# pecos/tps

Hardware: AMD Instinct MI355X
Metric: DG RHS evals/sec (MDOF/s) for 3D p=3 reacting cyl at 1/2/4/8 MI355X (higher is better)
Workload: dtype f64

## Files before the change

tps_amd/csrc/kernels.hpp:

```cpp
#ifndef TPSRHS_KERNELS_HPP_
#define TPSRHS_KERNELS_HPP_

#include <hip/hip_runtime.h>

#include <type_traits>

#include "basis.hpp"
#include "physics_dryair.hpp"

namespace tpsrhs {

#ifndef TPSRHS_MINW_GRAD
#define TPSRHS_MINW_GRAD 1
#endif
#ifndef TPSRHS_MINW_FLUX
#define TPSRHS_MINW_FLUX 3
#endif
#ifndef TPSRHS_NT_STORES
#define TPSRHS_NT_STORES 0
#endif
#ifndef TPSRHS_NO_MFMA
#define TPSRHS_NO_MFMA 0
#endif
#ifndef TPSRHS_FLUX_LATE
#define TPSRHS_FLUX_LATE 0
#endif
#ifndef TPSRHS_ABLATE
#define TPSRHS_ABLATE 0
#endif
constexpr int cmax(int a, int b) { return a > b ? a : b; }

#ifndef TPSRHS_STAMP
#define TPSRHS_STAMP 0
#endif
#if TPSRHS_STAMP
constexpr int NSTAMP = 16, STAMP_BLOCKS = 1 << 16;
static __device__ unsigned int g_stamp[STAMP_BLOCKS][NSTAMP];
struct Stamper {
  unsigned long long t0;
  unsigned int acc[NSTAMP];
  __device__ inline unsigned long long now() {
    unsigned long long t;
    __builtin_amdgcn_sched_barrier(0);
    asm volatile("s_memtime %0\n\ts_waitcnt lgkmcnt(0)" : "=s"(t)::"memory");
    __builtin_amdgcn_sched_barrier(0);
    return t;
  }
  __device__ inline void start() {
    for (int i = 0; i < NSTAMP; i++) acc[i] = 0;
    t0 = now();
  }
  __device__ inline void mark(int phase) {
    const unsigned long long t = now();
    acc[phase] += static_cast<unsigned int>(t - t0);
    t0 = t;
  }
  __device__ inline void flush() {
    if (threadIdx.x == 0 && blockIdx.x < STAMP_BLOCKS)
      for (int i = 0; i < NSTAMP; i++) g_stamp[blockIdx.x][i] = acc[i];
  }
};
#endif
#ifndef TPSRHS_DUMPF
#define TPSRHS_DUMPF 0
#endif
#if TPSRHS_DUMPF
constexpr int DUMPF_MAX = 1 << 22;
static __device__ double g_dumpf[DUMPF_MAX];
#endif
#if TPSRHS_STAMP == 1
#define STAMP_DECL Stamper stamper
#define STAMP_ARG , stamper
#define STAMP_PARAM , Stamper &stamper
#define STAMP_START() stamper.start()
#define STAMP(phase) stamper.mark(phase)
#define STAMP_FLUSH() stamper.flush()
#else
#define STAMP_DECL
#define STAMP_ARG
#define STAMP_PARAM
#define STAMP_START()
#define STAMP(phase)
#define STAMP_FLUSH()
#endif
#if TPSRHS_STAMP == 2
#define FSTAMP_DECL \
  Stamper stamper;  \
  stamper.start()
#define FSTAMP(phase) stamper.mark(phase)
#define FSTAMP_FLUSH() stamper.flush()
#else
#define FSTAMP_DECL
#define FSTAMP(phase)
#define FSTAMP_FLUSH()
#endif

static __constant__ Tables1D c_tab[2][2][TPSRHS_MAXORDER + 1];

__device__ inline const Tables1D &fresh_table(const Tables1D &ct) {
  typedef const Tables1D __attribute__((address_space(4))) *CP;
  const unsigned long long a = reinterpret_cast<unsigned long long>(&ct);
  unsigned lo = __builtin_amdgcn_readfirstlane(static_cast<unsigned>(a));
  unsigned hi = __builtin_amdgcn_readfirstlane(static_cast<unsigned>(a >> 32));
  asm volatile("" : "+s"(lo), "+s"(hi));
  return *(const Tables1D *)reinterpret_cast<CP>((static_cast<unsigned long long>(hi) << 32) | lo);
}

__device__ inline double ldsr(const double *p) { return *p; }

__device__ inline const double *field_ptr(const double *base, int k, int64_t stride) { return base + k * stride; }
__device__ inline double *field_ptr(double *base, int k, int64_t stride) { return base + k * stride; }

template <int BLOCK>
__device__ inline void block_sync() {
  if (BLOCK == 64) {
    __builtin_amdgcn_fence(__ATOMIC_RELEASE, "wavefront");
    __builtin_amdgcn_wave_barrier();
    __builtin_amdgcn_fence(__ATOMIC_ACQUIRE, "wavefront");
  } else {
    __syncthreads();
  }
}

template <int DIM_, int P_, int NC_ = 0>
struct Cfg {
  static constexpr int DIM = DIM_, P = P_, N1 = P_ + 1, NC = NC_;
  static constexpr int NPE = (DIM_ == 3) ? N1 * N1 * N1 : N1 * N1;
  static constexpr int NF = (DIM_ == 3) ? N1 * N1 : N1;
  static constexpr int Q1 = ((DIM_ - 1) + 2 * P_) / 2 + 1 + NC_;
  static constexpr int QV = P_ + 1 + NC_;
  static constexpr int NQV = (DIM_ == 3) ? QV * QV * QV : QV * QV;
  static constexpr int NQ = (DIM_ == 3) ? Q1 * Q1 : Q1;
  static constexpr int NW = (DIM_ == 3) ? Q1 * N1 : 1;
  static constexpr int NFACES = 2 * DIM_;
  static constexpr int NV = 1 << DIM_;
  static constexpr int BLOCK = (NC_ && DIM_ == 3 && P_ >= 2) ? 128 : ((NPE <= 64) ? 64 : ((NPE <= 128) ? 128 : 256));
  static constexpr int EPB = (DIM_ == 3 && NC_) ? (P_ == 3 ? 1 : 2)
                             : (DIM_ == 3 && P_ == 1) ? 3
                             : (DIM_ == 2 && NC_ && P_ == 1) ? 10
                                                             : BLOCK / NPE;
  static constexpr int NODES = EPB * NPE;
  static constexpr int PF = 2 * EPB;
  static constexpr int TN = PF * NF;
  static constexpr int TW = PF * NW;
  static constexpr int TQ = PF * NQ;
  static constexpr int LN = EPB * NF;
  static constexpr int Q_ROUNDS = (TQ + BLOCK - 1) / BLOCK;
  static_assert(DIM_ == 2 || Q_ROUNDS == 1, "3-D: one round of face quadrature points per direction pair");
  static_assert(!(DIM_ == 2 && NC_) || Q_ROUNDS == 1, "2-D Gauss-Lobatto pair: one round per direction pair");
  static constexpr int TQ2 = 2 * TQ;
  static constexpr int Q2_ROUNDS = (TQ2 + BLOCK - 1) / BLOCK;
};

template <class C>
struct Tab {
  double x[C::N1], w[C::N1], iw[C::N1], D[C::N1 * C::N1], b0[C::N1], b1[C::N1];
  double xq[C::Q1], wq[C::Q1], B[C::Q1 * C::N1];
  double xv[C::QV], wv[C::QV];
};

struct ForcingDev {
  int has_pg, nheat, nsponge, pad;
  double pg[3];
  struct Heat {
    double value, radius, len;
    double p1[3], axis[3];
  } heat[TPSRHS_MAXHEATSOURCES];
  struct Sponge {
    int type, pad;
    double normal[3], p0[3], pinit[3];
    double r1, r2, mult;
    double target[TPSRHS_MAXEQUATIONS];
    int mixed_out, n_plane;
    const int *plane_nodes;
    double *msum;
  } sponge[TPSRHS_MAXSPONGEZONES];
  const double *joule;
  int nps, pad2;
  struct Scalar {
    double x0[3], radius, value;
  } ps[TPSRHS_MAXPASSIVESCALARS];
// ... 1177 lines not shown
      for (int eq = 1; eq < NEQ; eq++) out[(eq - 1) * C::NQ] = fn[eq];
    }
    STAMP(8);
  }
}
template <class C, class PH, int D, int CD>
__device__ inline void lean_grad_chunk(const double *sJ, double *Tb, double *Wb, const Tab<C> &tab, const Tables1D &ct0,
                                       const double *n, double *gv, double *gn, int tid) {
  constexpr int NEQ = PH::NEQ, DIM = C::DIM, NVEL = PH::NVEL;
  const Tables1D &ct = fresh_table(ct0);
  trace_lines<C, D, NEQ>(sJ, Tb, ct, tid);
  block_sync<C::BLOCK>();
  interp1_lines<C, NEQ>(Tb, Wb, ct, tid);
  block_sync<C::BLOCK>();
  if (tid < C::TQ) {
    const int pf = tid / C::NQ, q = tid - pf * C::NQ;
    double bq[C::N1];
#pragma unroll
    for (int a = 0; a < C::N1; a++) bq[a] = tab.B[(q / C::Q1) * C::N1 + a];
#pragma unroll
    for (int k = 0; k < NEQ; k++) {
      const double val = interp2_point<C>(Tb + k * C::TN, Wb + k * C::TW, bq, pf, q);
      if (k >= 1 && k <= NVEL)
        gv[(k - 1) + CD * DIM] = val;
      else
        gn[k] += n[CD] * val;
    }
  }
  block_sync<C::BLOCK>();
}
template <class C, class PH, int D>
__device__ inline void lean_grad_dir(const MeshDev &m, const double *gradUp_q, bool node_on, unsigned node, double *gnext, double *sJ,
                                     double *Tb, double *Wb, const Tab<C> &tab, const Tables1D &ct, const double *n, double *gv,
                                     double *gn, int tid) {
  constexpr int NEQ = PH::NEQ;
  auto stage = [&](auto ctag) {
    constexpr int CD = decltype(ctag)::value;
    if (node_on) {
#pragma unroll
      for (int eq = 0; eq < NEQ; eq++) sJ[eq * C::NODES + tid] = gnext[eq];
      if (CD + 1 < C::DIM) {
        unsigned nq = node;
        int64_t stride = m.ndofs;
        asm volatile("" : "+v"(nq), "+s"(stride));
#pragma unroll
        for (int eq = 0; eq < NEQ; eq++) gnext[eq] = field_ptr(gradUp_q, (CD + 1) * NEQ + eq, stride)[nq];
      }
    }
    block_sync<C::BLOCK>();
    lean_grad_chunk<C, PH, D, CD>(sJ, Tb, Wb, tab, ct, n, gv, gn, tid);
  };
  stage(std::integral_constant<int, 0>());
  stage(std::integral_constant<int, 1>());
  stage(std::integral_constant<int, 2>());
}
template <class C, class PH>
__device__ inline void visc_phase_lean3d(const MeshDev &m, const int2 *sFI, typename PH::PRef prm0, int e0, const double *sU,
                                         const double *gradUp_q, bool node_on, unsigned node, double *sJ, double *Tb, double *Wb,
                                         const double *sV, const Tab<C> &tab, const Tables1D &ct, double *__restrict__ TB,
                                         int tid0 STAMP_PARAM) {
  constexpr int NEQ = PH::NEQ, DIM = C::DIM;
  static_assert(DIM == 3 && C::Q_ROUNDS == 1 && PH::NVEL == 3 && C::BLOCK == 64, "3-D, one wave, one round of face points per pair");
#pragma clang loop unroll(disable)
  for (int d = 0; d < DIM; d++) {
    typename PH::PRef prm = PH::relaunder(prm0);
    int tid = tid0;
    asm volatile("" : "+v"(tid));
    const int pf = tid / C::NQ, q = tid - pf * C::NQ;
    const int le = pf >> 1, s = pf & 1;
    const bool on = tid < C::TQ && (e0 + le) < m.ne;
    int nb = 0;
    double n[DIM] = {1.0, 0.0, 0.0};
    if (on) {
      double wq, Xq[DIM];
      nb = sFI[le * C::NFACES + 2 * d + s].x;
      face_geometry_rt<C>(d, &sV[le * C::NV * DIM], tab, s, q, n, wq, Xq);
    }
    const int np_lane = on ? PH::visc_passes(prm, nb) : 0;
    const int npass = (__ballot(np_lane == 2) != 0) ? 2 : ((__ballot(np_lane >= 1) != 0) ? 1 : 0);
    double *out = TB + static_cast<int64_t>((e0 + le) * C::NFACES + 2 * d + s) * ((NEQ - 1) * C::NQ) + q;
    if (on && np_lane == 0) {
#pragma unroll
      for (int eq = 1; eq < NEQ; eq++) out[(eq - 1) * C::NQ] = 0.0;
    }
#pragma clang loop unroll(disable)
    for (int pass = 0; pass < npass; pass++) {
      double u[NEQ];
#pragma unroll
      for (int k = 0; k < NEQ; k++) u[k] = 1.0;
      if (d == 0)
        visc_state_dir<C, PH, 0>(sU, Tb, Wb, tab, ct, u, tid);
      else if (d == 1)
        visc_state_dir<C, PH, 1>(sU, Tb, Wb, tab, ct, u, tid);
      else
        visc_state_dir<C, PH, 2>(sU, Tb, Wb, tab, ct, u, tid);
      STAMP(5);
      PH::clamp_species(u);
      double gnext[NEQ];
#pragma unroll
      for (int eq = 0; eq < NEQ; eq++) gnext[eq] = 0.0;
      if (node_on) {
        unsigned nq = node;
        int64_t stride = m.ndofs;
        asm volatile("" : "+v"(nq), "+s"(stride));
#pragma unroll
        for (int eq = 0; eq < NEQ; eq++) gnext[eq] = field_ptr(gradUp_q, eq, stride)[nq];
      }
      typename PH::ViscLean cf;
      if (pass < np_lane) {
        typename PH::PRef pq = PH::relaunder(prm);
        double Us[NEQ];
        typename PH::WallFlux w;
        PH::visc_pass_state(pq, nb, pass, u, n, Us, w);
        PH::visc_point_lean(pq, Us, w, cf);
      }
      STAMP(6);
      double gv[DIM * DIM], gn[NEQ];
#pragma unroll
      for (int k = 0; k < DIM * DIM; k++) gv[k] = 0.0;
#pragma unroll
      for (int eq = 0; eq < NEQ; eq++) gn[eq] = 0.0;
      if (d == 0)
        lean_grad_dir<C, PH, 0>(m, gradUp_q, node_on, node, gnext, sJ, Tb, Wb, tab, ct, n, gv, gn, tid);
      else if (d == 1)
        lean_grad_dir<C, PH, 1>(m, gradUp_q, node_on, node, gnext, sJ, Tb, Wb, tab, ct, n, gv, gn, tid);
      else
        lean_grad_dir<C, PH, 2>(m, gradUp_q, node_on, node, gnext, sJ, Tb, Wb, tab, ct, n, gv, gn, tid);
      STAMP(7);
      if (pass < np_lane) {
        double f[NEQ];
        PH::visc_normal_flux_lean(cf, gv, gn, n, f);
        if (nb >= 0) {
#pragma unroll
          for (int eq = 1; eq < NEQ; eq++) {
            if (TPSRHS_NT_STORES)
              __builtin_nontemporal_store(f[eq], &out[(eq - 1) * C::NQ]);
            else
              out[(eq - 1) * C::NQ] = f[eq];
          }
        } else if (pass == 0) {
#pragma unroll
          for (int eq = 1; eq < NEQ; eq++) out[(eq - 1) * C::NQ] = -0.5 * f[eq];
        } else {
#pragma unroll
          for (int eq = 1; eq < NEQ; eq++) out[(eq - 1) * C::NQ] -= 0.5 * f[eq];
        }
      }
      STAMP(8);
    }
    if (on && npass == 0) {
    }
  }
}
template <class C, class PH>
__device__ inline void visc_phase_2d(const MeshDev &m, const int2 *sFI, typename PH::PRef prm, int e0,
                                     const double *sU, const double *g, bool node_on, double *sJ, double *Tb,
                                     const double *sV, const Tab<C> &tab, const Tables1D &ct, double *__restrict__ TB,
                                     int tid, const double *sDist = nullptr) {
  static_assert(C::DIM == 2, "2-D only");
  constexpr int NEQ = PH::NEQ;
  typedef GradLds<C, PH> L;
  constexpr int G0 = PH::VISC_USES_GRAD_RHO ? 0 : 1, NG = NEQ - G0;
  double v[C::Q2_ROUNDS][L::NVF];
  auto chunk = [&](auto nfld_tag, const double *src, int v0) {
    constexpr int NF_ = decltype(nfld_tag)::value;
    trace_lines<C, 0, NF_>(src, Tb, ct, tid);
    trace_lines<C, 1, NF_>(src, Tb + L::CH * C::TN, ct, tid);
    block_sync<C::BLOCK>();
#pragma unroll
    for (int rd = 0; rd < C::Q2_ROUNDS; rd++) {
      int item = tid + rd * C::BLOCK;
      if (item < C::TQ2) {
        const int d = item / C::TQ;
        item -= d * C::TQ;
        const int pf = item / C::NQ, q = item - pf * C::NQ;
        const double *T = Tb + d * (L::CH * C::TN);
        double bq[C::N1];
#pragma unroll
        for (int a = 0; a < C::N1; a++) bq[a] = tab.B[q * C::N1 + a];
#pragma unroll
        for (int k = 0; k < NF_; k++) v[rd][v0 + k] = interp2_point<C>(T + k * C::TN, nullptr, bq, pf, q);
      }
    }
    block_sync<C::BLOCK>();
  };
  chunk(std::integral_constant<int, NEQ>(), sU, 0);
  FaceDist<C::Q2_ROUNDS> dq;
  dq.on = sDist != nullptr;
  if (sDist) {
    trace_lines<C, 0, 1>(sDist, Tb, ct, tid);
    trace_lines<C, 1, 1>(sDist, Tb + L::CH * C::TN, ct, tid);
    block_sync<C::BLOCK>();
#pragma unroll
    for (int rd = 0; rd < C::Q2_ROUNDS; rd++) {
      int item = tid + rd * C::BLOCK;
      dq.d[rd] = 0.0;
      if (item < C::TQ2) {
        const int d = item / C::TQ;
        item -= d * C::TQ;
        const int pf = item / C::NQ, q = item - pf * C::NQ;
        double bq[C::N1];
#pragma unroll
        for (int a = 0; a < C::N1; a++) bq[a] = tab.B[q * C::N1 + a];
        dq.d[rd] = interp2_point<C>(Tb + d * (L::CH * C::TN), nullptr, bq, pf, q);
      }
    }
    block_sync<C::BLOCK>();
  }
#pragma unroll
  for (int c = 1; c <= 2; c++) {
    const double *src;
    if constexpr (L::G_IN_LDS) {
      src = sJ + ((c - 1) * NEQ + G0) * C::NODES;
    } else {
      if (node_on) {
#pragma unroll
        for (int eq = G0; eq < NEQ; eq++) sJ[eq * C::NODES + tid] = g[eq + (c - 1) * NEQ];
      }
      block_sync<C::BLOCK>();
      src = sJ + G0 * C::NODES;
    }
    if (G0) {
#pragma unroll
      for (int rd = 0; rd < C::Q2_ROUNDS; rd++) v[rd][c * NEQ] = 0.0;
    }
    chunk(std::integral_constant<int, NG>(), src, c * NEQ + G0);
  }
  visc_points<C, PH, true>(m, sFI, prm, e0, 0, v, sV, tab, TB, tid, dq);
}
template <class C, class PH, int D>
__device__ inline void visc_traces_dir(const MeshDev &m, const int2 *sFI, typename PH::PRef prm, int e0,
                                       const double *sU, const double *g, bool node_on, double *sJ, double *Tb, double *Wb,
                                       const double *sV, const Tab<C> &tab, const Tables1D &ct, double *__restrict__ TB,
                                       int tid) {
  double v[C::Q_ROUNDS][GradLds<C, PH>::NVF];
  visc_interp_dir<C, PH, D>(sU, g, node_on, sJ, Tb, Wb, tab, ct, v, tid);
  visc_points<C, PH>(m, sFI, prm, e0, D, v, sV, tab, TB, tid);
}

template <class C, class PH>
__global__ __launch_bounds__(C::BLOCK, (C::NC && PH::HEAVY) ? 1 : PH::minw_grad(C::DIM, C::P, C::NC)) void k_gradient(MeshDev m, typename PH::KArg prm_k,
                                                       const double *__restrict__ U, const double *__restrict__ TA,
                                                       double *__restrict__ Upout, double *__restrict__ gradUp,
                                                       double *__restrict__ TB) {
  typename PH::PRef prm = PH::pref(prm_k);
  constexpr int NEQ = PH::NEQ, DIM = C::DIM;
  typedef GradLds<C, PH> L;
  const Tables1D &ct = c_tab[C::NC][DIM - 2][C::P];
  __shared__ Tab<C> tab;
  __shared__ double sV[C::EPB * C::NV * DIM];
  __shared__ double pool[L::TOTAL];
  double *sU = pool + L::O_U;
  double *sUp = pool + L::O_UP;
  double *sJ = pool + L::O_J;
  double *sW = pool + L::O_W;

  const int tid = threadIdx.x;
  const int lin = xcd_block(static_cast<int>(blockIdx.x), static_cast<int>(gridDim.x), m.reverse);
  const int bid = m.blocks ? m.blocks[lin] : lin;
  const int e0 = (TPSRHS_ABLATE & 512) ? (bid % 8) * C::EPB : bid * C::EPB;
  __shared__ int2 sFI[C::EPB * C::NFACES];
  STAMP_DECL;
  STAMP_START();
  const bool node_on = tid < C::NODES && (e0 + tid / C::NPE) < m.ne;
  const int le_n = tid / C::NPE, nd = tid - le_n * C::NPE;
  int idx[3] = {nd % C::N1, (nd / C::N1) % C::N1, nd / (C::N1 * C::N1)};
  double u[NEQ];
  if (node_on) {
    const unsigned n = static_cast<unsigned>(e0 + le_n) * C::NPE + nd;
#pragma unroll
    for (int eq = 0; eq < NEQ; eq++) u[eq] = field_ptr(U, eq, m.ndofs)[n];
  }
  load_face_info<C>(sFI, m, e0);
  load_tables<C>(tab, ct);
  load_vertices<C>(sV, m, e0);
  block_sync<C::BLOCK>();
  STAMP(0);
  NbTraces<C, NEQ> ta0, ta1, ta2;
  constexpr bool LATE = TPSRHS_GRAD_LATE && ((DIM == 3 && (!C::NC || TPSRHS_GRAD_LATE_NC) && !PH::HEAVY) || TPSRHS_GRAD_LATE_ALL);
  issue_neighbour_traces<C, 0, NEQ>(sFI, TA, 2 * NEQ * C::NF, NEQ, ta0, tid);
  if (!LATE) {
    issue_neighbour_traces<C, 1, NEQ>(sFI, TA, 2 * NEQ * C::NF, NEQ, ta1, tid);
    if (DIM == 3) issue_neighbour_traces<C, (DIM == 3 ? 2 : 0), NEQ>(sFI, TA, 2 * NEQ * C::NF, NEQ, ta2, tid);
  }
  if (node_on) {
    const unsigned n = static_cast<unsigned>(e0 + le_n) * C::NPE + nd;
    double up[NEQ];
    PH::prim(prm, u, up);
#pragma unroll
    for (int eq = 0; eq < NEQ; eq++) {
      sU[eq * C::NODES + tid] = u[eq];
      sUp[eq * C::NODES + tid] = up[eq];
      if (TPSRHS_NT_STORES)
        __builtin_nontemporal_store(up[eq], &field_ptr(Upout, eq, m.ndofs)[n]);
      else
        field_ptr(Upout, eq, m.ndofs)[n] = up[eq];
    }
  }
  block_sync<C::BLOCK>();
  STAMP(1);

  double g[NEQ * DIM];
#pragma unroll
  for (int k = 0; k < NEQ * DIM; k++) g[k] = 0.0;
  double inv_mass = 0.0;
  if constexpr (C::NC) {
    nc_volume_gradient<C, NEQ>(sUp, pool + L::O_V, sV, tab, ct, node_on, le_n, nd, tid, g);
  } else if (node_on) {
    double xi[DIM], J[DIM * DIM], A[DIM * DIM];
    double iwn = 1.0;
#pragma unroll
    for (int d = 0; d < DIM; d++) {
      xi[d] = tab.x[idx[d]];
      iwn *= tab.iw[idx[d]];
    }
    jacobian<DIM>(&sV[le_n * C::NV * DIM], xi, J);
    const double det = adjugate<DIM>(J, A);
    const double idet = fast_rcp(det);
    inv_mass = iwn * idet;
    double Dr[DIM][C::N1];
#pragma unroll
    for (int mm = 0; mm < DIM; mm++)
#pragma unroll
      for (int a = 0; a < C::N1; a++) Dr[mm][a] = tab.D[idx[mm] * C::N1 + a];
#pragma unroll
    for (int eq = 0; eq < NEQ; eq++) {
      double dr[DIM];
#pragma unroll
      for (int mm = 0; mm < DIM; mm++) {
        const int m2 = ((TPSRHS_ABLATE & 128) && DIM == 3) ? 2 : mm;
        const int sd = stride_of<C>(m2);
        const double *F = &sUp[eq * C::NODES + le_n * C::NPE + nd - idx[m2] * sd];
        double acc = 0.0;
#pragma unroll
        for (int a = 0; a < C::N1; a++) acc += Dr[mm][a] * ldsr(&F[a * sd]);
        dr[mm] = acc;
      }
#pragma unroll
      for (int d = 0; d < DIM; d++) {
        double s = 0.0;
#pragma unroll
        for (int mm = 0; mm < DIM; mm++) s += A[mm + d * DIM] * dr[mm];
        g[eq + d * NEQ] = s * idet;
      }
    }
  }

  STAMP(2);
  if (!(TPSRHS_ABLATE & 8)) {
    auto jump = [&](auto dtag) {
      constexpr int D = decltype(dtag)::value;
      if constexpr (C::NC) {
        nc_grad_jump<C, PH, D>(sFI, prm, sJ, pool + L::O_V, sV, tab, ct, node_on, le_n, idx, tid, g);
      } else {
        if (node_on) grad_jump_nodal<C, PH>(D, sFI, prm, sJ, sJ + NEQ * C::TN, sV, tab, le_n, idx, inv_mass, g);
        block_sync<C::BLOCK>();
      }
    };
    if (LATE) issue_neighbour_traces<C, 1, NEQ>(sFI, TA, 2 * NEQ * C::NF, NEQ, ta1, tid);
    trace_lines<C, 0, NEQ>(sUp, sJ, ct, tid);
    block_sync<C::BLOCK>();
    store_neighbour_traces<C, NEQ>(ta0, sJ, sJ + NEQ * C::TN, tid);
    block_sync<C::BLOCK>();
    jump(std::integral_constant<int, 0>());
    if (LATE && DIM == 3) issue_neighbour_traces<C, (DIM == 3 ? 2 : 0), NEQ>(sFI, TA, 2 * NEQ * C::NF, NEQ, ta2, tid);
    trace_lines<C, 1, NEQ>(sUp, sJ, ct, tid);
    block_sync<C::BLOCK>();
    store_neighbour_traces<C, NEQ>(ta1, sJ, sJ + NEQ * C::TN, tid);
    block_sync<C::BLOCK>();
    jump(std::integral_constant<int, 1>());
    if (DIM == 3) {
      trace_lines<C, (DIM == 3 ? 2 : 0), NEQ>(sUp, sJ, ct, tid);
      block_sync<C::BLOCK>();
      store_neighbour_traces<C, NEQ>(ta2, sJ, sJ + NEQ * C::TN, tid);
      block_sync<C::BLOCK>();
      jump(std::integral_constant<int, (DIM == 3 ? 2 : 0)>());
    }
  }
  if constexpr (C::NC) {
    if constexpr (C::NPE == 64 && C::BLOCK == 128 && !TPSRHS_NO_MFMA) {
      static_assert(L::V >= 64 * 17, "LDS buffer of the MFMA inverse mass");
      nc_apply_minv_mfma<C, NEQ * DIM>(m.minv, pool + L::O_V, node_on, e0, nd, tid, g);
    }
    else
      nc_apply_minv<C, NEQ * DIM>(m.minv, pool + L::O_V, node_on, e0 + le_n, le_n, nd, tid, g);
  }

  STAMP(3);
  if (node_on) {
    const unsigned n = static_cast<unsigned>(e0 + le_n) * C::NPE + nd;
#pragma unroll
    for (int k = 0; k < NEQ * DIM; k++) field_ptr(gradUp, k, m.ndofs)[n] = g[k];
    if constexpr (L::G_IN_LDS) {
#pragma unroll
      for (int k = 0; k < NEQ * DIM; k++) sJ[k * C::NODES + tid] = g[k];
    }
  }
  if (L::G_IN_LDS) block_sync<C::BLOCK>();
  STAMP(4);
  if constexpr (L::LEAN3D) {
    if (!(TPSRHS_ABLATE & 16)) {
      asm volatile("s_waitcnt vmcnt(0)" ::: "memory");
      const double *gq = gradUp;
      const unsigned node = static_cast<unsigned>(e0 + le_n) * C::NPE + nd;
      visc_phase_lean3d<C, PH>(m, sFI, prm, e0, sU, gq, node_on, node, sJ, sUp, sW, sV, tab, ct, TB, tid STAMP_ARG);
    }
    STAMP_FLUSH();
    return;
  }

  if (!(TPSRHS_ABLATE & 16)) {
    if constexpr (DIM == 2) {
      if constexpr (PH::HEAVY) {
        __shared__ double sDist[C::NODES];
        const bool ml_on = m.ml.distance != nullptr;
        if (ml_on) {
          if (tid < C::NODES)
            sDist[tid] = node_on ? m.ml.distance[static_cast<int64_t>(e0 + le_n) * C::NPE + nd] : 0.0;
          block_sync<C::BLOCK>();
        }
        visc_phase_2d<C, PH>(m, sFI, prm, e0, sU, g, node_on, sJ, sUp, sV, tab, ct, TB, tid, ml_on ? sDist : nullptr);
      } else {
        visc_phase_2d<C, PH>(m, sFI, prm, e0, sU, g, node_on, sJ, sUp, sV, tab, ct, TB, tid);
      }
    } else if constexpr (PH::TWO_STEP && C::Q_ROUNDS == 1 && !(TPSRHS_ABLATE & 256)) {
      visc_phase_heavy3d<C, PH>(m, sFI, prm, e0, sU, sJ, sUp, sW, sV, tab, ct, TB, tid STAMP_ARG);
    } else if constexpr (PH::HEAVY) {
#pragma clang loop unroll(disable)
      for (int d = 0; d < DIM; d++) {
        double v[C::Q_ROUNDS][L::NVF];
        if (d == 0)
          visc_interp_dir<C, PH, 0>(sU, g, node_on, sJ, sUp, sW, tab, ct, v, tid);
        else if (d == 1)
          visc_interp_dir<C, PH, 1>(sU, g, node_on, sJ, sUp, sW, tab, ct, v, tid);
        else
          visc_interp_dir<C, PH, (DIM == 3 ? 2 : 0)>(sU, g, node_on, sJ, sUp, sW, tab, ct, v, tid);
        visc_points<C, PH>(m, sFI, prm, e0, d, v, sV, tab, TB, tid);
      }
    } else {
      visc_traces_dir<C, PH, 0>(m, sFI, prm, e0, sU, g, node_on, sJ, sUp, sW, sV, tab, ct, TB, tid);
      visc_traces_dir<C, PH, 1>(m, sFI, prm, e0, sU, g, node_on, sJ, sUp, sW, sV, tab, ct, TB, tid);
      if (DIM == 3)
        visc_traces_dir<C, PH, (DIM == 3 ? 2 : 0)>(m, sFI, prm, e0, sU, g, node_on, sJ, sUp, sW, sV, tab, ct, TB, tid);
    }
  }
  STAMP_FLUSH();
}

template <class C, class PH>
__device__ inline void apply_forcing(const ForcingDev &f, typename PH::PRef prm, int64_t node, const double *X,
                                     const double *u, const typename PH::State &st, const double *gr, double *src) {
  constexpr int NEQ = PH::NEQ, DIM = C::DIM, NVEL = PH::NVEL;
  if (f.has_pg) {
    double gpv = 0.0;
#pragma unroll
    for (int d = 0; d < DIM; d++) {
      src[1 + d] -= f.pg[d];
      gpv -= st.vel[d] * f.pg[d];
      gpv -= st.p * gr[(1 + d) + d * NEQ];
    }
    src[1 + NVEL] += gpv;
  }
  if (f.nps > 0) {
    double up[NEQ];
    PH::prim(prm, u, up);
    for (int i = 0; i < f.nps; i++) {
      const ForcingDev::Scalar &ps = f.ps[i];
      double dist = 0.0;
#pragma unroll
      for (int d = 0; d < DIM; d++) dist += (X[d] - ps.x0[d]) * (X[d] - ps.x0[d]);
      if (sqrt(dist) < ps.radius) {
        double vel = 0.0;
#pragma unroll
        for (int d = 0; d < DIM; d++) vel += up[1 + d] * up[1 + d];
        vel = sqrt(vel);
        src[NEQ - 1] -= vel * (up[NEQ - 1] - up[0] * ps.value) / ps.radius;
      }
    }
  }
  for (int z = 0; z < f.nsponge; z++) {
    const ForcingDev::Sponge &sz = f.sponge[z];
    double dist_init = 0.0, dist_f = 0.0;
#pragma unroll
    for (int d = 0; d < DIM; d++) {
      dist_init -= sz.normal[d] * (X[d] - sz.pinit[d]);
      dist_f += sz.normal[d] * (X[d] - sz.p0[d]);
    }
    double sigma = 0.0;
    double tgt[NEQ];
#pragma unroll
    for (int eq = 0; eq < NEQ; eq++) tgt[eq] = sz.target[eq];
    if (sz.type == TPSRHS_SPONGE_PLANAR) {
      if (dist_init > 0.0 && dist_f > 0.0) {
        const double len = dist_f + dist_init;
        sigma = dist_init / len / len;
      }
    } else if constexpr (DIM == 3) {
      double t[3], R = 0.0;
#pragma unroll
      for (int d = 0; d < 3; d++) {
        t[d] = X[d] - sz.pinit[d] + dist_init * sz.normal[d];
        R += t[d] * t[d];
      }
      R = sqrt(R);
      if (dist_init > 0.0 && dist_f > 0.0 && R - sz.r1 > 0.0) {
        const double len = sz.r2 - sz.r1;
        sigma = (R - sz.r1) / len / len;
        double ur[3], uz[3], ut[3];
#pragma unroll
        for (int d = 0; d < 3; d++) {
          ur[d] = t[d] / R;
          uz[d] = sz.normal[d];
        }
        ut[0] = uz[1] * ur[2] - ur[1] * uz[2];
        ut[1] = uz[2] * ur[0] - uz[0] * ur[2];
        ut[2] = uz[0] * ur[1] - ur[0] * uz[1];
        const double M[9] = {ur[0], ur[1], ur[2], ut[0], ut[1], ut[2], uz[0], uz[1], uz[2]};
        const double c00 = M[4] * M[8] - M[5] * M[7], c01 = M[5] * M[6] - M[3] * M[8], c02 = M[3] * M[7] - M[4] * M[6];
        const double det = M[0] * c00 + M[1] * c01 + M[2] * c02;
        const double inv[9] = {c00, M[2] * M[7] - M[1] * M[8], M[1] * M[5] - M[2] * M[4],
                               c01, M[0] * M[8] - M[2] * M[6], M[2] * M[3] - M[0] * M[5],
                               c02, M[1] * M[6] - M[0] * M[7], M[0] * M[4] - M[1] * M[3]};
#pragma unroll
        for (int i = 0; i < 3; i++)
          tgt[1 + i] = (inv[3 * i] * sz.target[1] + inv[3 * i + 1] * sz.target[2] + inv[3 * i + 2] * sz.target[3]) / det;
      }
    }
    if (sigma > 0.0) {
      const double cs = PH::sound_speed(prm, sz.target);
      const double s = sigma * sz.mult;
#pragma unroll
      for (int eq = 0; eq < NEQ; eq++) src[eq] -= cs * s * (u[eq] - tgt[eq]);
    }
  }
  for (int h = 0; h < f.nheat; h++) {
    const ForcingDev::Heat &hs = f.heat[h];
    double proj = 0.0, Xr[DIM];
#pragma unroll
    for (int d = 0; d < DIM; d++) {
      Xr[d] = X[d] - hs.p1[d];
      proj += Xr[d] * hs.axis[d];
    }
    double r2 = 0.0;
#pragma unroll
    for (int d = 0; d < DIM; d++) {
      const double r = Xr[d] - proj * hs.axis[d];
      r2 += r * r;
    }
    if (sqrt(r2) < hs.radius && proj > 0.0 && proj < hs.len) src[DIM + 1] += hs.value;
  }
  if (f.joule) {
    const double heating = f.joule[node];
    if (heating > 0.0) {
      src[NVEL + 1] += heating;
      if (PH::TWO_TEMPERATURE) src[NEQ - 1] += heating;
    }
  }
}
// ... 862 lines not shown
```

tps_amd/csrc/physics_plasma.hpp:

```cpp
#ifndef TPSRHS_PHYSICS_PLASMA_HPP_
#define TPSRHS_PHYSICS_PLASMA_HPP_

#include <hip/hip_runtime.h>

#include "physics_dryair.hpp"

namespace tpsrhs {

#pragma clang fp reciprocal(on)

constexpr double kRgas = 8.3144598;
constexpr double kAvogadro = 6.0221409e+23;
constexpr double kBoltz = kRgas / kAvogadro;
constexpr double kEps0 = 8.8541878128e-12;
constexpr double kQe = 1.60218e-19;
constexpr double kMolarQe = kQe * kAvogadro;
constexpr double kPi = 3.14159265358979323846;
constexpr double kXeps = 1.0e-30;

struct TableDev {
  int n, x_log, f_log, pad;
  const double *x, *a, *b;
  double x0, inv_dx;
};
// ... 49 lines not shown
    int it = first;
    const int step = count / 2;
    it += step;
    if (xe > t.x[it]) {
      first = ++it;
      count -= step + 1;
    } else {
      count = step;
    }
  }
  first = max(1, min(t.n - 1, first));
  return first - 1;
}
template <class TD>
__device__ inline double table_eval(const TD &t, double xe) {
  const int idx = table_interval(t, xe);
  const double xt = t.x_log ? flog(xe) : xe;
  double ft = t.a[idx] + t.b[idx] * xt;
  if (t.f_log) ft = fexp(ft);
  return ft;
}

namespace coll {
struct Arg {
  double ln, inv2;
};
__device__ inline Arg arg(double Tp) {
  Arg a;
  a.ln = flog(Tp);
  const double r = fast_rcp(Tp);
  a.inv2 = r * r;
  return a;
}
__device__ inline double cfit(double c0, double c1, double c2, double c3, const Arg &a) {
  const double L = flog_pos(1.0 + c1 * fexp<false>(c2 * a.ln));
  const double v = c0 * fexp<false>(c3 * flog_pos(L)) * a.inv2;
  return (L > 0.0) ? v : ((L == 0.0) ? 0.0 : v);
}
template <int N>
__device__ inline void cfit_n(const double (&c)[N][4], const Arg &a, double (&out)[N]) {
  double t[N], E[N], w[N], L[N], lL[N], u[N], P[N];
#pragma unroll
  for (int i = 0; i < N; i++) t[i] = c[i][2] * a.ln;
  fexp_n<N>(t, E);
#pragma unroll
  for (int i = 0; i < N; i++) w[i] = 1.0 + c[i][1] * E[i];
  flog_pos_n<N>(w, L);
  flog_pos_n<N>(L, lL);
#pragma unroll
  for (int i = 0; i < N; i++) u[i] = c[i][3] * lL[i];
  fexp_n<N>(u, P);
#pragma unroll
  for (int i = 0; i < N; i++) {
    const double v = c[i][0] * P[i] * a.inv2;
    out[i] = (L[i] > 0.0) ? v : ((L[i] == 0.0) ? 0.0 : v);
  }
}
__device__ inline double att11(const Arg &a) { return cfit(0.2150, 5.2194, 1.0472, 1.2435, a); }
__device__ inline double att12(const Arg &a) { return cfit(0.0991, 7.4684, 1.0155, 1.1536, a); }
__device__ inline double att13(const Arg &a) { return cfit(0.0616, 7.8271, 0.9452, 1.1105, a); }
__device__ inline double att14(const Arg &a) { return cfit(0.0308, 13.9567, 0.9511, 1.1803, a); }
__device__ inline double att15(const Arg &a) { return cfit(0.0232, 13.7888, 0.9148, 1.1532, a); }
__device__ inline double rep22(const Arg &a) { return cfit(0.4128, 1.2436, 1.1830, 1.0123, a); }
__device__ inline double rep23(const Arg &a) { return cfit(0.2203, 1.8832, 1.2059, 0.9851, a); }
__device__ inline double rep24(const Arg &a) { return cfit(0.1323, 2.7248, 1.2129, 0.9847, a); }
__constant__ static double c_coulomb[2][2][5][4] = {
    {{{0.2150, 5.2194, 1.0472, 1.2435}, {0.0991, 7.4684, 1.0155, 1.1536}, {0.0616, 7.8271, 0.9452, 1.1105},
      {0.0308, 13.9567, 0.9511, 1.1803}, {0.0232, 13.7888, 0.9148, 1.1532}},
     {{0, 0, 0, 0}, {0.2423, 4.6796, 1.3290, 1.1279}, {0.1221, 8.7542, 1.3875, 1.1110}, {0.0619, 18.2538, 1.4341, 1.1618},
      {0, 0, 0, 0}}},
    {{{0.3904, 0.9100, 1.1025, 1.0544}, {0.1547, 1.6597, 1.1725, 0.9792}, {0.0814, 2.5815, 1.1948, 0.9570},
      {0.0683, 1.9774, 1.2033, 0.8264}, {0.0346, 4.5177, 1.2132, 0.9294}},
     {{0, 0, 0, 0}, {0.4128, 1.2436, 1.1830, 1.0123}, {0.2203, 1.8832, 1.2059, 0.9851}, {0.1323, 2.7248, 1.2129, 0.9847},
      {0, 0, 0, 0}}}};
__device__ inline double ArAr11(double lnT) { return 2.2910e-18 * fexp(-0.3032 * lnT); }
__device__ inline double ArAr22(double T) { return 1.7e-18 * fast_rsqrt(fast_sqrt(T)); }
__device__ inline double iArAr22(double sqrtT) { return fast_sqrt(sqrtT) * (1.0 / 1.7e-18); }
__device__ inline double ArAr1P11(double lnT) { return 4.574321e-18 * fexp(-0.1805 * lnT); }
__device__ inline double eAr1r(int r, double logT) {
  const double C[5][9] = {
      {6.36254140e-18, 1.84835040e-18, -5.87727093e-18, 3.20023027e-18, -8.50509054e-19, 1.28163820e-19,
       -1.11712910e-20, 5.25649382e-22, -1.03296658e-23},
      {1.91338172e-17, 5.45418129e-18, -1.78361685e-17, 9.75657946e-18, -2.61115722e-18, 3.98310268e-19,
       -3.53503678e-20, 1.70375066e-21, -3.45211955e-23},
      {3.04685398e-17, 8.39750994e-18, -2.88132528e-17, 1.60147037e-17, -4.34837891e-18, 6.73136845e-19,
       -6.06704580e-20, 2.97216168e-21, -6.12760944e-23},
      {3.90777949e-17, 1.04696956e-17, -3.73774204e-17, 2.10610498e-17, -5.79029566e-18, 9.07573157e-19,
       -8.28466766e-20, 4.11188110e-21, -8.59225098e-23},
      {4.41333290e-17, 1.15696010e-17, -4.25651305e-17, 2.42442440e-17, -6.73359258e-18, 1.06641697e-18,
       -9.83933863e-20, 4.93775812e-21, -1.04362372e-22}};
  double fit = C[r - 1][0] * fast_rcp(logT), pw = 1.0;
#pragma unroll
  for (int k = 1; k < 9; k++) {
    fit += C[r - 1][k] * pw;
    pw *= logT;
  }
  return fit;
}
template <int NR>
__device__ inline void eAr1r_n(double logT, double (&fit)[NR]) {
  static_assert(NR <= 5, "five fits");
  constexpr double C[5][9] = {
      {6.36254140e-18, 1.84835040e-18, -5.87727093e-18, 3.20023027e-18, -8.50509054e-19, 1.28163820e-19,
       -1.11712910e-20, 5.25649382e-22, -1.03296658e-23},
      {1.91338172e-17, 5.45418129e-18, -1.78361685e-17, 9.75657946e-18, -2.61115722e-18, 3.98310268e-19,
       -3.53503678e-20, 1.70375066e-21, -3.45211955e-23},
      {3.04685398e-17, 8.39750994e-18, -2.88132528e-17, 1.60147037e-17, -4.34837891e-18, 6.73136845e-19,
       -6.06704580e-20, 2.97216168e-21, -6.12760944e-23},
      {3.90777949e-17, 1.04696956e-17, -3.73774204e-17, 2.10610498e-17, -5.79029566e-18, 9.07573157e-19,
       -8.28466766e-20, 4.11188110e-21, -8.59225098e-23},
      {4.41333290e-17, 1.15696010e-17, -4.25651305e-17, 2.42442440e-17, -6.73359258e-18, 1.06641697e-18,
       -9.83933863e-20, 4.93775812e-21, -1.04362372e-22}};
  const double il = fast_rcp(logT);
#pragma unroll
  for (int r = 0; r < NR; r++) fit[r] = C[r][0] * il;
  double pw = 1.0;
#pragma unroll
  for (int k = 1; k < 9; k++) {
#pragma unroll
    for (int r = 0; r < NR; r++) fit[r] += C[r][k] * pw;
    pw *= logT;
  }
}
}

#ifndef TPSRHS_PLASMA_MINW_FLUX
#define TPSRHS_PLASMA_MINW_FLUX 2
#endif
#ifndef TPSRHS_PLASMA_MINW_GRAD3
#define TPSRHS_PLASMA_MINW_GRAD3 2
#endif
#ifndef TPSRHS_PLASMA_MINW_GRAD_LEAN
#define TPSRHS_PLASMA_MINW_GRAD_LEAN 3
#endif
enum { TRANSPORT_CONSTANT = 0, TRANSPORT_ARGON_MINIMAL = 1, TRANSPORT_ARGON_MIXTURE = 2 };

template <int DIM_, int NVEL_, int NSP_, bool AMBI, bool TWOT, int TRANSPORT>
struct PlasmaPhys {
  static constexpr int DIM = DIM_, NVEL = NVEL_, NSP = NSP_;
  static constexpr int NACTIVE = AMBI ? NSP_ - 2 : NSP_ - 1;
  static constexpr int NEQ = NVEL_ + 2 + NACTIVE + (TWOT ? 1 : 0);
  static constexpr int IE = NSP_ - 2, IB = NSP_ - 1;
  static constexpr int ITH = NVEL_ + 1, ITE = NEQ - 1;
  static constexpr bool HAS_SOURCE = true;
  static constexpr bool TWO_TEMPERATURE = TWOT;
  static constexpr int MAX_ORDER = 4;
  static constexpr bool HAS_NR_BC = false;
  static constexpr bool LES = false;
  static constexpr bool HAS_MIXED_OUT = false;
  static constexpr bool VISC_USES_GRAD_RHO = true;
  static constexpr bool AXISYM = NVEL_ > DIM_;
  static constexpr int MINW_GRAD = (NSP_ > 3) ? 1 : TPSRHS_PLASMA_MINW_GRAD3;
  static constexpr bool LEAN_TRACE = (NSP_ == 3) && (DIM_ == 3);
  static constexpr bool LAUNDER_FLUX = false;
  static constexpr int minw_grad(int dim, int p, int nc) {
    return (LEAN_TRACE && dim == 3 && !nc && p <= 3) ? TPSRHS_PLASMA_MINW_GRAD_LEAN : MINW_GRAD;
  }
  static constexpr int MINW_FLUX = (NSP_ > 6 || (NSP_ > 3 && DIM_ == 3)) ? 1 : TPSRHS_PLASMA_MINW_FLUX;
  typedef PlasmaParams<NSP_> Params;
  typedef const Params *KArg;
  typedef const Params __attribute__((address_space(4))) &PRef;
  typedef const BcDev __attribute__((address_space(4))) &BcRef;
  __device__ static inline PRef pref(KArg k) { return *(const Params __attribute__((address_space(4))) *)k; }
  __device__ static inline PRef relaunder(PRef p) {
    const unsigned long long a = reinterpret_cast<unsigned long long>(&p);
    unsigned lo = __builtin_amdgcn_readfirstlane(static_cast<unsigned>(a));
    unsigned hi = __builtin_amdgcn_readfirstlane(static_cast<unsigned>(a >> 32));
    asm volatile("" : "+s"(lo), "+s"(hi));
    return *reinterpret_cast<const Params __attribute__((address_space(4))) *>((static_cast<unsigned long long>(hi) << 32) | lo);
  }
  struct Transport {};

  struct State {
    double ir, k, p, pe, Th, Te, c;
    double vel[NVEL];
    double n[NSP];
  };

  __device__ static inline void number_densities(PRef p, const double *U, double *n) {
#pragma unroll
    for (int sp = 0; sp < NSP; sp++) n[sp] = 0.0;
#pragma unroll
    for (int sp = 0; sp < NACTIVE; sp++) n[sp] = U[NVEL + 2 + sp] * p.imw[sp];
    double rhoB = U[0];
#pragma unroll
    for (int sp = 0; sp < NACTIVE; sp++) rhoB -= p.mw[sp] * n[sp];
    if (AMBI) {
      double ne = 0.0;
#pragma unroll
      for (int sp = 0; sp < NACTIVE; sp++) ne += p.charge[sp] * n[sp];
      ne = fmax(ne, 0.0);
      n[IE] = ne;
      rhoB -= ne * p.mw[IE];
    }
    n[IB] = rhoB * p.imw[IB];
  }
  __device__ static inline double heavies_cv(PRef p, const double *n) {
    double c = 0.0;
#pragma unroll
    for (int sp = 0; sp < NACTIVE; sp++)
      if (sp != IE) c += n[sp] * p.cv[sp];
    return c + n[IB] * p.cv[IB];
  }
  __device__ static inline double heavies_n(const double *n) {
    double nh = 0.0;
#pragma unroll
    for (int sp = 0; sp < NACTIVE; sp++)
      if (sp != IE) nh += n[sp];
    return nh + n[IB];
  }
  __device__ static inline State make_state(PRef p, const double *U) {
    State s;
    number_densities(p, U, s.n);
    s.ir = fast_rcp(U[0]);
    double m2 = 0.0;
#pragma unroll
    for (int d = 0; d < NVEL; d++) {
      m2 += U[1 + d] * U[1 + d];
      s.vel[d] = U[1 + d] * s.ir;
    }
    s.k = m2 * s.ir;
    const double chv = heavies_cv(p, s.n);
    double ctot = chv;
    if (!TWOT) ctot += s.n[IE] * p.cv[IE];
    double e = U[ITH];
#pragma unroll
    for (int sp = 0; sp < NSP - 2; sp++) e -= s.n[sp] * p.eform[sp];
    double Th = -0.5 * s.k + e;
    if (TWOT) Th -= U[ITE];
    s.Th = Th * fast_rcp(ctot);
    s.Te = TWOT ? U[ITE] * fast_rcp(s.n[IE] * p.cv[IE]) : s.Th;
    const double nh = heavies_n(s.n);
    s.pe = s.n[IE] * kRgas * s.Te;
    s.p = kRgas * (nh * s.Th + s.n[IE] * s.Te);
    const double gamma = 1.0 + nh * kRgas * fast_rcp(chv);
    s.c = fast_sqrt(gamma * s.p * s.ir);
    return s;
  }
  __device__ static inline double pressure(PRef p, const double *U) { return make_state(p, U).p; }

  __device__ static inline void prim(PRef p, const double *U, double *Up) {
    const State s = make_state(p, U);
    Up[0] = U[0];
#pragma unroll
    for (int d = 0; d < NVEL; d++) Up[1 + d] = s.vel[d];
    Up[ITH] = s.Th;
#pragma unroll
    for (int sp = 0; sp < NACTIVE; sp++) Up[NVEL + 2 + sp] = s.n[sp];
    if (TWOT) Up[ITE] = s.Te;
  }
  __device__ static inline void clamp_species(double *U) {
#pragma unroll
    for (int sp = 0; sp < NACTIVE; sp++) U[NVEL + 2 + sp] = fmax(U[NVEL + 2 + sp], 0.0);
  }
  __device__ static inline double max_char_speed(PRef, const double *, const State &s) {
    return fast_sqrt(s.k * s.ir) + s.c;
  }
  __device__ static inline double max_char_speed(PRef p, const double *U) {
    return max_char_speed(p, U, make_state(p, U));
  }
  __device__ static inline double sound_speed(PRef p, const double *U) {
    return make_state(p, U).c;
  }

  __device__ static inline void conv_flux_n(PRef p, const double *U, const State &s, const double *n,
                                            double *Fn) {
    double un = 0.0;
#pragma unroll
    for (int d = 0; d < DIM; d++) un += s.vel[d] * n[d];
    Fn[0] = U[0] * un;
#pragma unroll
    for (int i = 0; i < NVEL; i++) Fn[1 + i] = U[1 + i] * un + (i < DIM ? s.p * n[i] : 0.0);
    Fn[ITH] = un * (U[ITH] + s.p);
#pragma unroll
    for (int sp = 0; sp < NACTIVE; sp++) Fn[NVEL + 2 + sp] = U[NVEL + 2 + sp] * un;
    if (TWOT) Fn[ITE] = (U[ITE] + s.pe) * un;
  }
  __device__ static inline void lax_friedrichs(PRef p, const double *U1, const double *U2, const double *n,
                                               double *F) {
    const State s1 = make_state(p, U1), s2 = make_state(p, U2);
    const double lam = fmax(max_char_speed(p, U1, s1), max_char_speed(p, U2, s2));
    double f1[NEQ], f2[NEQ];
    conv_flux_n(p, U1, s1, n, f1);
    conv_flux_n(p, U2, s2, n, f2);
    double nm = 0.0;
#pragma unroll
    for (int d = 0; d < DIM; d++) nm += n[d] * n[d];
    const double hl = 0.5 * lam * fast_sqrt(nm);
#pragma unroll
    for (int eq = 0; eq < NEQ; eq++) F[eq] = 0.5 * (f1[eq] + f2[eq]) - hl * (U2[eq] - U1[eq]);
  }

  __device__ static inline void riemann(PRef p, const double *U1, const double *U2, const double *n, double *F) {
    lax_friedrichs(p, U1, U2, n, F);
  }
  __device__ static inline void riemann_bc(PRef p, BcRef, const double *U1, const double *Ug,
                                           const double *n, double *F) {
    lax_friedrichs(p, U1, Ug, n, F);
  }
  struct Species {
    double X[NSP], Y[NSP], n[NSP], ntot, intot;
  };
  __device__ static inline Species species(PRef p, const double *U) {
    Species q;
    const double ir = fast_rcp(U[0]);
    double n = 0.0, ne = 0.0, Yb = 1.0;
// ... 1202 lines not shown
```

Baseline: 12550.

## Add single-wave-per-hex lean viscous face phase for 3D argon plasma

Adds a specialized viscous face-flux path for 3D single-temperature minimal-argon plasma where one 64-lane wave handles one hex. It interpolates the state and gradient traces to the face through a two-stage LDS tensor-product contraction. Gradient loads for the next component are issued with scalar base addresses and overlapped with the current contraction. The aim is to cut LDS traffic, sync overhead and register pressure compared with the general lean3d path, at the cost of more specialized code paths and extra barriers per stage.

```diff
diff --git a/tps_amd/csrc/kernels.hpp b/tps_amd/csrc/kernels.hpp
--- a/tps_amd/csrc/kernels.hpp
+++ b/tps_amd/csrc/kernels.hpp
@@ -27,6 +27,9 @@
 #endif
 #ifndef TPSRHS_ABLATE
 #define TPSRHS_ABLATE 0
+#endif
+#ifndef TPSRHS_LEAN_GENERAL
+#define TPSRHS_LEAN_GENERAL 0
 #endif
 constexpr int cmax(int a, int b) { return a > b ? a : b; }
 
@@ -1510,6 +1513,238 @@
     }
   }
 }
+template <class C>
+struct LeanLane {
+  unsigned lane;
+  unsigned tw;
+  unsigned ir, iw;
+  unsigned pw, pb;
+  static constexpr int FPR = C::BLOCK / C::LN;
+  static_assert(C::EPB == 1 && C::DIM == 3 && C::BLOCK == 64 && C::BLOCK % C::LN == 0 && C::TQ <= C::BLOCK, "one hex per wave");
+  __device__ explicit LeanLane(unsigned t) : lane(t) {
+    tw = (t / C::LN) * C::TN + t % C::LN;
+    const unsigned fld = t / (C::PF * C::N1), r = t % (C::PF * C::N1), pf1 = r / C::N1, jb = r % C::N1;
+    ir = fld * C::TN + pf1 * C::NF + C::N1 * jb;
+    iw = fld * C::TW + pf1 * C::NW + jb;
+    const unsigned tq = t < C::TQ ? t : C::TQ - 1, pf = tq / C::NQ, q = tq - pf * C::NQ;
+    pw = pf * C::NW + (q % C::Q1) * C::N1;
+    pb = (q / C::Q1) * C::N1;
+  }
+  template <int D>
+  __device__ unsigned trace_src() const {
+    const unsigned ln = lane % C::LN;
+    return (lane / C::LN) * C::NODES + (ln % C::N1) * stride_of<C>(tan_a<C>(D)) + (ln / C::N1) * stride_of<C>(tan_b<C>(D));
+  }
+};
+template <class C, int D, int NFLD>
+__device__ inline void lean1_lines(const double *F, double *Tb, double *Wb, const Tables1D &ct, const LeanLane<C> &ll, unsigned src) {
+  constexpr int sd = stride_of<C>(D), FPR = LeanLane<C>::FPR, ROUNDS = (NFLD + FPR - 1) / FPR;
+  static_assert(NFLD * C::PF * C::N1 <= C::BLOCK, "interp1_lines: one round");
+#pragma unroll
+  for (int r = 0; r < ROUNDS; r++) {
+    if ((r + 1) * FPR <= NFLD || ll.lane < static_cast<unsigned>((NFLD - r * FPR) * C::LN)) {
+      const double *f = F + r * FPR * C::NODES + src;
+      double t0 = 0.0, t1 = 0.0;
+#pragma unroll
+      for (int i = 0; i < C::N1; i++) {
+        const double v = ldsr(&f[i * sd]);
+        t0 += ct.b0[i] * v;
+        t1 += ct.b1[i] * v;
+      }
+      double *t = Tb + r * FPR * C::TN + ll.tw;
+      t[0] = t0;
+      t[C::NF] = t1;
+    }
+    if (r + 1 < ROUNDS) __builtin_amdgcn_sched_barrier(0);
+  }
+  block_sync<C::BLOCK>();
+  if (ll.lane < static_cast<unsigned>(NFLD * C::PF * C::N1)) {
+    const double *t = Tb + ll.ir;
+    double v[C::N1];
+#pragma unroll
+    for (int ja = 0; ja < C::N1; ja++) v[ja] = ldsr(&t[ja]);
+    double *w = Wb + ll.iw;
+#pragma unroll
+    for (int qa = 0; qa < C::Q1; qa++) {
+      double acc = 0.0;
+#pragma unroll
+      for (int ja = 0; ja < C::N1; ja++) acc += ct.B[qa * C::N1 + ja] * v[ja];
+      w[qa * C::N1] = acc;
+    }
+  }
+  block_sync<C::BLOCK>();
+}
+template <class C>
+__device__ inline double lean1_point(const double *Wb, int k, const double *bq, const LeanLane<C> &ll) {
+  const double *w = Wb + k * C::TW + ll.pw;
+  double acc = 0.0;
+#pragma unroll
+  for (int jb = 0; jb < C::N1; jb++) acc += bq[jb] * ldsr(&w[jb]);
+  return acc;
+}
+template <class C>
+__device__ inline unsigned long long lean1_grad_base(const double *gradUp_q, int e0) {
+  unsigned es = __builtin_amdgcn_readfirstlane(e0);
+  asm volatile("" : "+s"(es));
+  return reinterpret_cast<unsigned long long>(gradUp_q) + static_cast<unsigned long long>(es) * (C::NPE * sizeof(double));
+}
+template <int NEQ>
+__device__ inline void lean1_issue_grad(unsigned long long &a, unsigned long long step, unsigned lane, double *gnext) {
+  typedef const double __attribute__((address_space(1))) *GP;
+#pragma unroll
+  for (int eq = 0; eq < NEQ; eq++) {
+    asm volatile("" : "+s"(a));
+    gnext[eq] = reinterpret_cast<GP>(a)[lane];
+    a += step;
+  }
+}
+template <class C, class PH, int D>
+__device__ inline void lean1_grad_dir(unsigned long long ga, unsigned long long gstep, bool node_on, double *gnext, double *sJ,
+                                      double *Tb, double *Wb, const Tab<C> &tab, const Tables1D &ct0, const double *n, double *gv,
+                                      double *gn, const LeanLane<C> &ll) {
+  constexpr int NEQ = PH::NEQ, DIM = C::DIM, NVEL = PH::NVEL;
+  const unsigned src = ll.template trace_src<D>();
+  auto stage = [&](auto ctag) {
+    constexpr int CD = decltype(ctag)::value;
+    if (node_on) {
+#pragma unroll
+      for (int eq = 0; eq < NEQ; eq++) sJ[eq * C::NODES + ll.lane] = gnext[eq];
+      if (CD + 1 < DIM) lean1_issue_grad<NEQ>(ga, gstep, ll.lane, gnext);
+    }
+    block_sync<C::BLOCK>();
+    const Tables1D &ct = fresh_table(ct0);
+    lean1_lines<C, D, NEQ>(sJ, Tb, Wb, ct, ll, src);
+    double bq[C::N1];
+#pragma unroll
+    for (int a = 0; a < C::N1; a++) bq[a] = tab.B[ll.pb + a];
+#pragma unroll
+    for (int k = 0; k < NEQ; k++) {
+      const double val = lean1_point<C>(Wb, k, bq, ll);
+      if (k >= 1 && k <= NVEL)
+        gv[(k - 1) + CD * DIM] = val;
+      else if (CD == 0)
+        gn[k] = 0.0 + n[CD] * val;
+      else
+        gn[k] += n[CD] * val;
+    }
+#pragma unroll
+    for (int k = 0; k < NEQ; k++) {
+      if (k >= 1 && k <= NVEL)
+        asm volatile("" : "+v"(gv[(k - 1) + CD * DIM]));
+      else
+        asm volatile("" : "+v"(gn[k]));
+    }
+    block_sync<C::BLOCK>();
+  };
+  stage(std::integral_constant<int, 0>());
+  stage(std::integral_constant<int, 1>());
+  stage(std::integral_constant<int, 2>());
+}
+template <class C, class PH, int D>
+__device__ inline void lean1_state_dir(const double *sU, double *Tb, double *Wb, const Tab<C> &tab, const Tables1D &ct0, double *u,
+                                       const LeanLane<C> &ll) {
+  const Tables1D &ct = fresh_table(ct0);
+  lean1_lines<C, D, PH::NEQ>(sU, Tb, Wb, ct, ll, ll.template trace_src<D>());
+  double bq[C::N1];
+#pragma unroll
+  for (int a = 0; a < C::N1; a++) bq[a] = tab.B[ll.pb + a];
+#pragma unroll
+  for (int k = 0; k < PH::NEQ; k++) u[k] = lean1_point<C>(Wb, k, bq, ll);
+  block_sync<C::BLOCK>();
+}
+template <class C, class PH>
+__device__ inline void visc_phase_lean1(const MeshDev &m, const int2 *sFI, typename PH::PRef prm0, int e0, const double *sU,
+                                        const double *gradUp_q, bool node_on0, double *sJ, double *Tb, double *Wb,
+                                        const double *sV, const Tab<C> &tab, const Tables1D &ct, double *__restrict__ TB,
+                                        int tid0 STAMP_PARAM) {
+  constexpr int NEQ = PH::NEQ, DIM = C::DIM;
+  static_assert(DIM == 3 && C::Q_ROUNDS == 1 && PH::NVEL == 3 && C::BLOCK == 64 && C::EPB == 1, "3-D, one wave = one hex");
+  const bool node_on = __builtin_amdgcn_readfirstlane(node_on0) != 0;
+#pragma clang loop unroll(disable)
+  for (int d = 0; d < DIM; d++) {
+    typename PH::PRef prm = PH::relaunder(prm0);
+    int tid = tid0;
+    asm volatile("" : "+v"(tid));
+    const int pf = tid / C::NQ, q = tid - pf * C::NQ;
+    const int le = pf >> 1, s = pf & 1;
+    const bool on = tid < C::TQ && (e0 + le) < m.ne;
+    int nb = 0;
+    double n[DIM] = {1.0, 0.0, 0.0};
+    if (on) {
+      double wq, Xq[DIM];
+      nb = sFI[le * C::NFACES + 2 * d + s].x;
+      face_geometry_rt<C>(d, &sV[le * C::NV * DIM], tab, s, q, n, wq, Xq);
+    }
+    const int np_lane = on ? PH::visc_passes(prm, nb) : 0;
+    const int npass = (__ballot(np_lane == 2) != 0) ? 2 : ((__ballot(np_lane >= 1) != 0) ? 1 : 0);
+    double *out = TB + static_cast<int64_t>((e0 + le) * C::NFACES + 2 * d + s) * ((NEQ - 1) * C::NQ) + q;
+    if (on && np_lane == 0) {
+#pragma unroll
+      for (int eq = 1; eq < NEQ; eq++) out[(eq - 1) * C::NQ] = 0.0;
+    }
+#pragma clang loop unroll(disable)
+    for (int pass = 0; pass < npass; pass++) {
+      double u[NEQ];
+      int tid1 = tid0;
+      asm volatile("" : "+v"(tid1));
+      const LeanLane<C> ll(static_cast<unsigned>(tid1) & (C::BLOCK - 1));
+      if (d == 0)
+        lean1_state_dir<C, PH, 0>(sU, Tb, Wb, tab, ct, u, ll);
+      else if (d == 1)
+        lean1_state_dir<C, PH, 1>(sU, Tb, Wb, tab, ct, u, ll);
+      else
+        lean1_state_dir<C, PH, 2>(sU, Tb, Wb, tab, ct, u, ll);
+      STAMP(5);
+      PH::clamp_species(u);
+      double gnext[NEQ];
+      unsigned long long ga = lean1_grad_base<C>(gradUp_q, e0);
+      const unsigned long long gstep = static_cast<unsigned long long>(m.ndofs) * sizeof(double);
+      if (node_on) {
+        lean1_issue_grad<NEQ>(ga, gstep, ll.lane, gnext);
+      } else {
+#pragma unroll
+        for (int eq = 0; eq < NEQ; eq++) gnext[eq] = 0.0;
+      }
+      typename PH::ViscLean cf;
+      if (pass < np_lane) {
+        typename PH::PRef pq = PH::relaunder(prm);
+        double Us[NEQ];
+        typename PH::WallFlux w;
+        PH::visc_pass_state(pq, nb, pass, u, n, Us, w);
+        PH::visc_point_lean(pq, Us, w, cf);
+      }
+      STAMP(6);
+      double gv[DIM * DIM], gn[NEQ];
+      if (d == 0)
+        lean1_grad_dir<C, PH, 0>(ga, gstep, node_on, gnext, sJ, Tb, Wb, tab, ct, n, gv, gn, ll);
+      else if (d == 1)
+        lean1_grad_dir<C, PH, 1>(ga, gstep, node_on, gnext, sJ, Tb, Wb, tab, ct, n, gv, gn, ll);
+      else
+        lean1_grad_dir<C, PH, 2>(ga, gstep, node_on, gnext, sJ, Tb, Wb, tab, ct, n, gv, gn, ll);
+      STAMP(7);
+      if (pass < np_lane) {
+        double f[NEQ];
+        PH::visc_normal_flux_lean(cf, gv, gn, n, f);
+        if (nb >= 0) {
+#pragma unroll
+          for (int eq = 1; eq < NEQ; eq++) {
+            if (TPSRHS_NT_STORES)
+              __builtin_nontemporal_store(f[eq], &out[(eq - 1) * C::NQ]);
+            else
+              out[(eq - 1) * C::NQ] = f[eq];
+          }
+        } else if (pass == 0) {
+#pragma unroll
+          for (int eq = 1; eq < NEQ; eq++) out[(eq - 1) * C::NQ] = -0.5 * f[eq];
+        } else {
+#pragma unroll
+          for (int eq = 1; eq < NEQ; eq++) out[(eq - 1) * C::NQ] -= 0.5 * f[eq];
+        }
+      }
+      STAMP(8);
+    }
+  }
+}
 template <class C, class PH>
 __device__ inline void visc_phase_2d(const MeshDev &m, const int2 *sFI, typename PH::PRef prm, int e0,
                                      const double *sU, const double *g, bool node_on, double *sJ, double *Tb,
@@ -1761,7 +1996,10 @@
       asm volatile("s_waitcnt vmcnt(0)" ::: "memory");
       const double *gq = gradUp;
       const unsigned node = static_cast<unsigned>(e0 + le_n) * C::NPE + nd;
-      visc_phase_lean3d<C, PH>(m, sFI, prm, e0, sU, gq, node_on, node, sJ, sUp, sW, sV, tab, ct, TB, tid STAMP_ARG);
+      if constexpr (PH::LEAN_ONE_HEX && C::EPB == 1 && C::BLOCK % C::LN == 0 && !TPSRHS_ABLATE && !TPSRHS_LEAN_GENERAL)
+        visc_phase_lean1<C, PH>(m, sFI, prm, e0, sU, gq, node_on, sJ, sUp, sW, sV, tab, ct, TB, tid STAMP_ARG);
+      else
+        visc_phase_lean3d<C, PH>(m, sFI, prm, e0, sU, gq, node_on, node, sJ, sUp, sW, sV, tab, ct, TB, tid STAMP_ARG);
     }
     STAMP_FLUSH();
     return;
diff --git a/tps_amd/csrc/physics_plasma.hpp b/tps_amd/csrc/physics_plasma.hpp
--- a/tps_amd/csrc/physics_plasma.hpp
+++ b/tps_amd/csrc/physics_plasma.hpp
@@ -225,6 +225,7 @@
   static constexpr bool AXISYM = NVEL_ > DIM_;
   static constexpr int MINW_GRAD = (NSP_ > 3) ? 1 : TPSRHS_PLASMA_MINW_GRAD3;
   static constexpr bool LEAN_TRACE = (NSP_ == 3) && (DIM_ == 3);
+  static constexpr bool LEAN_ONE_HEX = LEAN_TRACE && !TWOT && TRANSPORT == TRANSPORT_ARGON_MINIMAL;
   static constexpr bool LAUNDER_FLUX = false;
   static constexpr int minw_grad(int dim, int p, int nc) {
     return (LEAN_TRACE && dim == 3 && !nc && p <= 3) ? TPSRHS_PLASMA_MINW_GRAD_LEAN : MINW_GRAD;
```

Measured after the change: 12940, median of 6. +3.1%, better.
